# stm233/image-compression-for-machine

Hardware: AMD Instinct MI355X
Metric: images/sec (256x256) cnn-hyperprior (WACNN) training step (higher is better)
Workload: dtype f32; 1 GPU; cnn (WACNN N=192 M=320) train step, lambda=0.0067 MSE, batch 16/GPU synthetic 256x256, Adam lr 1e-4 + aux Adam, clip 1.0; global_batch=16, parallelism=dp1

## Files before the change

### image-compression-for-machine_amd/csrc/conv_wgrad.hip

```cpp
#include <algorithm>
#include <cmath>
#include <cstdlib>
#include "icm_common.h"

namespace icm {

#define WG_MAX_TAPS 32

int wgrad_wino_plan(const icm_wgrad_args& a, int nproblems, int* nsplit_out, int* nchunks_out);
int launch_wgrad_wino(const icm_wgrad_args* arr, int n, int nsplit, int nchunks, float* const* ws, float* const* dbias_ws,
                      hipStream_t stream);

#define WG_MAXG 32
struct WgPtrs {
  const float* gs;
  const float* gb;
  float* ws;
  float* dbias_ws;
};
struct WgDesc {
  WgPtrs g[WG_MAXG];
  long long gs_bs;
  PatchGeom pg;
  int Ca, OH, OW, act_s;
// ... 392 lines not shown
      const int a = a0 + ta * 32 + (r & 3) + 8 * (r >> 2) + 4 * h;
      if (a < d.Ca && b < pg.C)
        G.ws[(((long long)split * d.ntaps + tap) * d.Ca + a) * pg.C + b] = acc[i][r];
    }
    __builtin_amdgcn_sched_barrier(0);
  }
}

template <int TA, int TB, int WA, int WB, bool V4>
__global__ __launch_bounds__(512, 2) void wgrad_dma1_kernel(const WgDesc d) {
  extern __shared__ __attribute__((aligned(16))) float smem[];
  static_assert(TA == 3 * WA && TB == 3 * WB && (WA * WB == 1 || WA * WB == 2 || WA * WB == 4), "3 x 3 tiles per wave");
  constexpr int WK = 8 / (WA * WB);
  const PatchGeom& pg = d.pg;
  const int npx = 1 << d.lgNPX, grow = V4 ? 64 : npx + 1, brow = V4 ? 64 : pg.CS;
  const int gs_sz = TA * 32 * grow, gb_sz = TB * 32 * brow;
  const int bufsz = gs_sz + gb_sz;
  const int tid = threadIdx.x, lane = tid & 63;
  const int wave = __builtin_amdgcn_readfirstlane(tid >> 6);
  const WgPtrs G = d.g[blockIdx.y];
  int bid = blockIdx.x;
  if (d.xcd_order) bid = xcd_block_id();
  const int at = bid % d.natile; bid /= d.natile;
  const int bt = bid % d.nbtile;
  const int split = bid / d.nbtile;
  const int a0 = at * TA * 32, b0 = bt * TB * 32;
  const int niter = (d.ntiles - split + d.nsplit - 1) / d.nsplit;
  const int TWm = (1 << d.lgTW) - 1, THm = (1 << d.lgTH) - 1;
  const int OHW = d.OH * d.OW;
  const long long HW = (long long)pg.H * pg.W;
  const float* zero = icm_zero_page + lane;
  const float* zero4 = icm_zero_page + 4 * lane;

  auto stage = [&](int it) {
    int q = split + it * d.nsplit;
    const int tx_i = q % d.tiles_x; q /= d.tiles_x;
    const int ty_i = q % d.tiles_y;
    const int tn_i = q / d.tiles_y;
    const int ox0 = tx_i << d.lgTW, oy0 = ty_i << d.lgTH, n0 = tn_i << d.lgTI;
    float* gsT = smem + (it & 1) * bufsz;
    float* gbP = gsT + gs_sz;
    const int tx = lane & TWm, ty = (lane >> d.lgTW) & THm, ti = lane >> (d.lgTW + d.lgTH);
    const int n = n0 + ti, oy = oy0 + ty, ox = ox0 + tx;
    const bool pv = n < pg.N && oy < d.OH && ox < d.OW;
    const float* abase = G.gs + ((long long)n * d.gs_bs + oy * d.OW + ox);
    const float* bbase = G.gb + ((long long)n * pg.bs + oy * pg.W + ox);
    if constexpr (V4) {
      const int s = lane >> 4, q = lane & 15;
      for (int i = wave; i < (TA + TB) * 8; i += 8) {
        const bool isa = i < TA * 8;
        const int r = (isa ? i : i - TA * 8) * 4 + s;
        const int px = ((q - (r & 15)) & 15) * 4;
        const int tx4 = px & TWm, ty4 = (px >> d.lgTW) & THm, ti4 = px >> (d.lgTW + d.lgTH);
        const int n4 = n0 + ti4, oy4 = oy0 + ty4, ox4 = ox0 + tx4;
        const bool pv4 = n4 < pg.N && oy4 < d.OH && ox4 < d.OW;
        const float* src;
        if (isa) {
          const int a = a0 + r;
          src = (pv4 && a < d.Ca) ? G.gs + ((long long)n4 * d.gs_bs + (long long)a * OHW + oy4 * d.OW + ox4) : zero4;
        } else {
          const int c = b0 + r;
          src = (pv4 && c < pg.C) ? G.gb + ((long long)n4 * pg.bs + (long long)c * HW + oy4 * pg.W + ox4) : zero4;
        }
        __builtin_amdgcn_global_load_lds(src, (isa ? gsT : gbP) + (isa ? i : i - TA * 8) * 256, 16, 0, 0);
      }
    } else if (lane < npx) {
      for (int r = wave; r < TA * 32; r += 8) {
        const int a = a0 + r;
        __builtin_amdgcn_global_load_lds((pv && a < d.Ca) ? abase + (long long)a * OHW : zero, gsT + r * grow, 4, 0, 0);
      }
      for (int r = wave; r < TB * 32; r += 8) {
        const int c = b0 + r;
        __builtin_amdgcn_global_load_lds((pv && c < pg.C) ? bbase + (long long)c * HW : zero, gbP + r * pg.CS, 4, 0, 0);
      }
    }
  };

  const int h = lane >> 5, l31 = lane & 31;
  const int wk = wave % WK, wsp = wave / WK;
  const int wa = wsp / WB, wb = wsp % WB;
  int boffs[3];
#pragma unroll
  for (int u = 0; u < 3; ++u) boffs[u] = ((wb * 3 + u) * 32 + l31) * brow + (V4 ? 0 : h);
  const int rot = 4 * (l31 & 15) + h;
  f32x16 acc[9];
#pragma unroll
  for (int i = 0; i < 9; ++i)
#pragma unroll
    for (int r = 0; r < 16; ++r) acc[i][r] = 0.0f;
  float bsum[3] = {0.0f, 0.0f, 0.0f};
  const int nkp = npx >> 1;

  stage(0);
  asm volatile("s_waitcnt vmcnt(0)" ::: "memory");
  __syncthreads();
  for (int it = 0; it < niter; ++it) {
    if (it + 1 < niter) stage(it + 1);
    const float* gsT = smem + (it & 1) * bufsz;
    const float* gbP = gsT + gs_sz;
    const float* arow = gsT + (wa * 3 * 32 + l31) * grow + (V4 ? 0 : h);
    float avA[3], bvA[3], avB[3], bvB[3];
    auto fetch = [&](float (&av)[3], float (&bv)[3], int kn) {
      const int col = V4 ? ((2 * kn + rot) & 63) : 2 * kn;
#pragma unroll
      for (int u = 0; u < 3; ++u) av[u] = arow[u * 32 * grow + col];
#pragma unroll
      for (int u = 0; u < 3; ++u) bv[u] = gbP[boffs[u] + col];
    };
    auto mma = [&](const float (&av)[3], const float (&bv)[3]) {
#pragma unroll
      for (int ta = 0; ta < 3; ++ta)
#pragma unroll
        for (int tb = 0; tb < 3; ++tb)
          acc[ta * 3 + tb] = __builtin_amdgcn_mfma_f32_32x32x2f32(av[ta], bv[tb], acc[ta * 3 + tb], 0, 0, 0);
#pragma unroll
      for (int u = 0; u < 3; ++u) bsum[u] += av[u];
    };
    fetch(avA, bvA, wk);
    for (int kp = wk; kp < nkp; kp += 2 * WK) {
      fetch(avB, bvB, min(kp + WK, nkp - 1));
      mma(avA, bvA);
      fetch(avA, bvA, min(kp + 2 * WK, nkp - 1));
      if (kp + WK < nkp) mma(avB, bvB);
    }
    asm volatile("s_waitcnt vmcnt(0)" ::: "memory");
    __syncthreads();
  }
  constexpr int SET = 9 * 16 * 64;
  constexpr int SLOTS = (WK - 1) < 2 ? (WK - 1) : 2;
  float* red = smem + wsp * SLOTS * SET;
#pragma unroll
  for (int r0 = 1; r0 < WK; r0 += SLOTS) {
    if (wk >= r0 && wk < r0 + SLOTS) {
      float* dst = red + (wk - r0) * SET;
#pragma unroll
      for (int i = 0; i < 9; ++i)
#pragma unroll
        for (int r = 0; r < 16; ++r) dst[(i * 16 + r) * 64 + lane] = acc[i][r];
    }
    __syncthreads();
    if (wk == 0) {
      for (int k = 0; k < SLOTS && r0 + k < WK; ++k)
#pragma unroll
        for (int i = 0; i < 9; ++i)
#pragma unroll
          for (int r = 0; r < 16; ++r) acc[i][r] += red[k * SET + (i * 16 + r) * 64 + lane];
    }
    __syncthreads();
  }
  if (G.dbias_ws != nullptr && bt == 0) {
    float* bred = smem;
    if (wb == 0) {
#pragma unroll
      for (int u = 0; u < 3; ++u) {
        const float sfull = bsum[u] + __shfl_xor(bsum[u], 32, 64);
        if (h == 0) bred[(wa * WK + wk) * 96 + u * 32 + l31] = sfull;
      }
    }
    __syncthreads();
    if (wb == 0 && wk == 0 && h == 0) {
#pragma unroll
      for (int u = 0; u < 3; ++u) {
        float t = 0.0f;
        for (int k = 0; k < WK; ++k) t += bred[(wa * WK + k) * 96 + u * 32 + l31];
        const int a = a0 + (wa * 3 + u) * 32 + l31;
        if (a < d.Ca) G.dbias_ws[(long long)split * d.Ca + a] = t;
      }
    }
  }
  if (wk != 0) return;
#pragma unroll
  for (int i = 0; i < 9; ++i) {
    const int ta = wa * 3 + i / 3, tb = wb * 3 + i % 3;
    const int b = b0 + tb * 32 + l31;
#pragma unroll
    for (int r = 0; r < 16; ++r) {
      const int a = a0 + ta * 32 + (r & 3) + 8 * (r >> 2) + 4 * h;
      if (a < d.Ca && b < pg.C) G.ws[((long long)split * d.Ca + a) * pg.C + b] = acc[i][r];
    }
    __builtin_amdgcn_sched_barrier(0);
  }
}

template <int TA, int TB, int NACC>
__global__ __launch_bounds__(512, 2) void wgrad_kernel(const WgDesc d) {
  extern __shared__ __attribute__((aligned(16))) float smem[];
  const PatchGeom& pg = d.pg;
  const int npx = 1 << d.lgNPX, grow = npx + 1;
  const int gs_sz = TA * 32 * grow, gb_sz = TB * 32 * pg.CS;
  const int bufsz = gs_sz + gb_sz;
  const int tid = threadIdx.x, lane = tid & 63, wave = tid >> 6;
  const bool loader = wave >= 4;
  const WgPtrs G = d.g[blockIdx.y];

  int bid = blockIdx.x;
  if (d.xcd_order) bid = xcd_block_id();
  const int at = bid % d.natile; bid /= d.natile;
  const int bt = bid % d.nbtile; bid /= d.nbtile;
  const int tg = bid % d.ngroups;
  const int split = bid / d.ngroups;
  const int a0 = at * TA * 32, b0 = bt * TB * 32, t0 = tg * d.tpg;
  const int nt = min(d.tpg, d.ntaps - t0);
  const int TWm = (1 << d.lgTW) - 1, THm = (1 << d.lgTH) - 1;
  const int niter = (d.ntiles - split + d.nsplit - 1) / d.nsplit;

  if (loader) {
    wgrad_loader<TA, TB>(d, G, smem, tid, lane, wave, a0, b0, split, niter, bt, tg);
    return;
  }

  const int h = lane >> 5, l31 = lane & 31;
  const int ntile = nt * TA * TB;
  int boffs[NACC];
  int tsel[NACC];
#pragma unroll
  for (int i = 0; i < NACC; ++i) {
    const int q = wave + 4 * i;
    const int qq = q < ntile ? q : 0;
    const int tap = qq / (TA * TB), rem = qq % (TA * TB);
    const int ta = rem / TB, tb = rem % TB;
    tsel[i] = q < ntile ? ta : -1;
    boffs[i] = (tb * 32 + l31) * pg.CS + d.tapoff[t0 + tap] + h * d.po_h;
  }
  f32x16 acc[NACC];
#pragma unroll
  for (int i = 0; i < NACC; ++i)
#pragma unroll
    for (int r = 0; r < 16; ++r) acc[i][r] = 0.0f;

  const int pe_lane = d.pe[lane & 31];
  constexpr bool kPerAcc = (TA * TB == 16);
  static_assert(kPerAcc ? (NACC == 4 && TA == 4) : (4 % (TA * TB) == 0), "tile -> A-row mapping");
  constexpr int NA = kPerAcc ? TA : 1;
  const int ta_w = kPerAcc ? 0 : (wave % (TA * TB)) / TB;
  __syncthreads();
  const int nkp = npx >> 1;
  for (int it = 0; it < niter; ++it) {
    const float* gsT = smem + (it & 1) * bufsz;
    const float* gbP = gsT + gs_sz;
    const float* arow = gsT + (ta_w * 32 + l31) * grow + h;
    float avA[NA], bvA[NACC], avB[NA], bvB[NACC];
    auto fetch = [&](float (&av)[NA], float (&bv)[NACC], int kn) {
      const int po = __builtin_amdgcn_readlane(pe_lane, kn);
#pragma unroll
      for (int u = 0; u < NA; ++u) av[u] = arow[u * 32 * grow + 2 * kn];
#pragma unroll
      for (int i = 0; i < NACC; ++i) bv[i] = gbP[boffs[i] + po];
    };
    auto mma = [&](const float (&av)[NA], const float (&bv)[NACC]) {
#pragma unroll
      for (int i = 0; i < NACC; ++i)
        acc[i] = __builtin_amdgcn_mfma_f32_32x32x2f32(av[kPerAcc ? i : 0], bv[i], acc[i], 0, 0, 0);
    };
    fetch(avA, bvA, 0);
    for (int kp = 0; kp < nkp; kp += 2) {
      fetch(avB, bvB, kp + 1);
      mma(avA, bvA);
#pragma unroll
      for (int i = 0; i < NACC; ++i) {
        __builtin_amdgcn_sched_group_barrier(0x008, 1, 0);
        __builtin_amdgcn_sched_group_barrier(0x002, 2, 0);
        __builtin_amdgcn_sched_group_barrier(0x100, 2, 0);
      }
      fetch(avA, bvA, min(kp + 2, nkp - 1));
      mma(avB, bvB);
#pragma unroll
      for (int i = 0; i < NACC; ++i) {
        __builtin_amdgcn_sched_group_barrier(0x008, 1, 0);
        __builtin_amdgcn_sched_group_barrier(0x002, 2, 0);
        __builtin_amdgcn_sched_group_barrier(0x100, 2, 0);
      }
    }
    __syncthreads();
  }

#pragma unroll
  for (int i = 0; i < NACC; ++i) {
    if (tsel[i] < 0) continue;
    const int q = wave + 4 * i;
    const int tap = t0 + q / (TA * TB), rem = q % (TA * TB);
    const int ta = rem / TB, tb = rem % TB;
    const int b = b0 + tb * 32 + l31;
#pragma unroll
    for (int r = 0; r < 16; ++r) {
      const int a = a0 + ta * 32 + (r & 3) + 8 * (r >> 2) + 4 * h;
      if (a < d.Ca && b < pg.C)
        G.ws[(((long long)split * d.ntaps + tap) * d.Ca + a) * pg.C + b] = acc[i][r];
    }
    __builtin_amdgcn_sched_barrier(0);
  }
}

struct RedPtrs {
  const float* ws;
  float* dw;
  const float* dbias_ws;
  float* dbias;
  int accum, accum_bias;
  int dw_ld;
};
struct RedDesc {
  RedPtrs g[WG_MAXG];
  int Ca, Cb, ntaps, nsplit, nsplit_bias, nwblocks, vec4;
  int wino;
};
__global__ __launch_bounds__(256) void wgrad_reduce_kernel(const RedDesc d) {
  __shared__ __attribute__((aligned(16))) float tile[WG_MAX_TAPS][257];
  const RedPtrs G = d.g[blockIdx.y];
  const int Ca = d.Ca, ntaps = d.ntaps, nsplit = d.nsplit;
  if ((int)blockIdx.x >= d.nwblocks) {
    if (!G.dbias) return;
    float* part = &tile[0][0];
    const int pl = threadIdx.x & 15, sl = threadIdx.x >> 4;
    const int a = ((int)blockIdx.x - d.nwblocks) * 16 + pl;
    float s = 0.0f;
    if (a < Ca)
      for (int k = sl; k < d.nsplit_bias; k += 16) s += G.dbias_ws[(long long)k * Ca + a];
    part[sl * 16 + pl] = s;
    __syncthreads();
    if (sl == 0 && a < Ca) {
      float t = part[pl];
#pragma unroll
      for (int u = 1; u < 16; ++u) t += part[u * 16 + pl];
      if (G.accum_bias) t += G.dbias[a];
      G.dbias[a] = t;
    }
    return;
  }
  const long long CaCb = (long long)Ca * d.Cb;
  const long long slab = CaCb * ntaps;
  if (d.vec4) {
    f32x4* part = reinterpret_cast<f32x4*>(&tile[0][0]);
    const int pl = threadIdx.x & 15, sl = threadIdx.x >> 4;
    const long long ab = ((long long)blockIdx.x * 16 + pl) * 4;
    f32x4 s = f32x4{0.0f, 0.0f, 0.0f, 0.0f};
    if (ab < CaCb) {
      const float* p = G.ws + ab;
      int k = sl;
      for (; k + 7 * 16 < nsplit; k += 8 * 16) {
        f32x4 v[8];
#pragma unroll
        for (int u = 0; u < 8; ++u) v[u] = *reinterpret_cast<const f32x4*>(p + (long long)(k + 16 * u) * slab);
#pragma unroll
        for (int u = 0; u < 8; ++u) s += v[u];
      }
      for (; k < nsplit; k += 16) s += *reinterpret_cast<const f32x4*>(p + (long long)k * slab);
    }
    part[sl * 16 + pl] = s;
    __syncthreads();
    if (sl == 0 && ab < CaCb) {
      f32x4 t = part[pl];
#pragma unroll
      for (int u = 1; u < 16; ++u) t += part[u * 16 + pl];
      const long long ar = ab / d.Cb;
      f32x4* o = reinterpret_cast<f32x4*>(G.dw + (G.dw_ld == d.Cb ? ab : ar * G.dw_ld + (ab - ar * d.Cb)));
      if (G.accum) t += *o;
      *o = t;
    }
    return;
  }
  const int pl = threadIdx.x & 63, tl = threadIdx.x >> 6;
  const long long ab0 = (long long)blockIdx.x * 64;
  const long long ab = ab0 + pl;
  const bool valid = ab < CaCb;
  for (int t = tl; t < ntaps; t += 8) {
    const int t2 = t + 4;
    float sa = 0.0f, sb = 0.0f;
    if (valid) {
      const float* pa = G.ws + (long long)t * CaCb + ab;
      const float* pb = G.ws + (long long)(t2 < ntaps ? t2 : t) * CaCb + ab;
      for (int k = 0; k < nsplit; k += 8) {
        float va[8], vb[8];
#pragma unroll
        for (int u = 0; u < 8; ++u) {
          va[u] = (k + u < nsplit) ? pa[(long long)(k + u) * slab] : 0.0f;
          vb[u] = (k + u < nsplit) ? pb[(long long)(k + u) * slab] : 0.0f;
        }
        sa += ((va[0] + va[1]) + (va[2] + va[3])) + ((va[4] + va[5]) + (va[6] + va[7]));
        sb += ((vb[0] + vb[1]) + (vb[2] + vb[3])) + ((vb[4] + vb[5]) + (vb[6] + vb[7]));
      }
    }
    tile[t][pl] = sa;
    if (t2 < ntaps) tile[t2][pl] = sb;
  }
  __syncthreads();
  const int nv = (int)min((long long)64, CaCb - ab0);
  if (d.wino) {
    for (int e = threadIdx.x; e < nv * 9; e += 256) {
      const int abl = e / 9, t = e - abl * 9;
      const int p = t / 3, q = t - p * 3;
      float col[4];
#pragma unroll
      for (int i = 0; i < 4; ++i) {
        const float u0 = tile[i * 4 + 0][abl], u1 = tile[i * 4 + 1][abl], u2 = tile[i * 4 + 2][abl], u3 = tile[i * 4 + 3][abl];
        col[i] = q == 0 ? u0 + 0.5f * (u1 + u2) : (q == 1 ? 0.5f * (u1 - u2) : 0.5f * (u1 + u2) + u3);
      }
      float v = p == 0 ? col[0] + 0.5f * (col[1] + col[2]) : (p == 1 ? 0.5f * (col[1] - col[2]) : 0.5f * (col[1] + col[2]) + col[3]);
      const long long abg = ab0 + abl, ar = abg / d.Cb;
      float* o = G.dw + (ar * G.dw_ld + (abg - ar * d.Cb)) * 9 + t;
      if (G.accum) v += *o;
      *o = v;
    }
    return;
  }
  if (G.dw_ld == d.Cb) {
    float* o = G.dw + ab0 * ntaps;
    for (int e = threadIdx.x; e < nv * ntaps; e += 256) {
      const int abl = e / ntaps, t = e - abl * ntaps;
      float v = tile[t][abl];
      if (G.accum) v += o[e];
      o[e] = v;
    }
  } else {
    for (int e = threadIdx.x; e < nv * ntaps; e += 256) {
      const int abl = e / ntaps, t = e - abl * ntaps;
      const long long abg = ab0 + abl, ar = abg / d.Cb;
      float* o = G.dw + (ar * G.dw_ld + (abg - ar * d.Cb)) * ntaps + t;
      float v = tile[t][abl];
      if (G.accum) v += *o;
      *o = v;
    }
  }
}

enum WgFamily {
  WG_GENERAL,
  WG_T33,
  WG_T33_TAPW,
  WG_TAP9,
  WG_TAP25,
  WG_DMA1,
};
typedef void (*WgKernel)(const WgDesc);
struct WgVariant {
  WgFamily fam;
  int ta, tb, nacc;
  int tpg;
  bool halves;
  int lds_kb;
  WgKernel fn, fn_v4;
};
static const WgVariant kWgVariants[] = {
     {WG_GENERAL, 2, 1, 7, 14, true, 150, wgrad_kernel<2, 1, 7>, nullptr},
     {WG_GENERAL, 2, 2, 9, 9, false, 150, wgrad_kernel<2, 2, 9>, nullptr},
     {WG_GENERAL, 4, 4, 4, 1, false, 150, wgrad_kernel<4, 4, 4>, nullptr},
     {WG_T33, 3, 3, 9, 1, false, 160, wgrad_t33_kernel<3, 3, 1, 1>, nullptr},
     {WG_T33, 6, 6, 9, 1, false, 160, wgrad_t33_kernel<6, 6, 2, 2>, nullptr},
     {WG_T33, 3, 6, 9, 1, false, 160, wgrad_t33_kernel<3, 6, 1, 2>, nullptr},
     {WG_T33, 6, 3, 9, 1, false, 160, wgrad_t33_kernel<6, 3, 2, 1>, nullptr},
     {WG_T33_TAPW, 3, 3, 9, 4, false, 160, wgrad_t33_kernel<3, 3, 1, 1, true>, nullptr},
     {WG_TAP9, 3, 3, 9, 9, false, 160, wgrad_tap9_kernel<3, 3>, nullptr},
     {WG_TAP9, 2, 2, 9, 9, false, 160, wgrad_tap9_kernel<2, 2>, nullptr},
     {WG_TAP25, 3, 1, 10, 25, false, 160, wgrad_tap9_kernel<3, 1, 3>, nullptr},
     {WG_DMA1, 6, 6, 9, 1, false, 160, wgrad_dma1_kernel<6, 6, 2, 2, false>, wgrad_dma1_kernel<6, 6, 2, 2, true>},
     {WG_DMA1, 3, 6, 9, 1, false, 160, wgrad_dma1_kernel<3, 6, 1, 2, false>, wgrad_dma1_kernel<3, 6, 1, 2, true>},
     {WG_DMA1, 6, 3, 9, 1, false, 160, wgrad_dma1_kernel<6, 3, 2, 1, false>, wgrad_dma1_kernel<6, 3, 2, 1, true>},
     {WG_DMA1, 3, 3, 9, 1, false, 160, wgrad_dma1_kernel<3, 3, 1, 1, false>, wgrad_dma1_kernel<3, 3, 1, 1, true>},
};
constexpr int WG_NVARIANTS = sizeof(kWgVariants) / sizeof(kWgVariants[0]);
static int g_force_variant = -1, g_force_xcd = -1;

struct WgPlan {
  int variant, tpg;
  int lgTW, lgTH, lgTI, lgNPX, PH, PW, PP, CS;
  int tiles_x, tiles_y, tiles_n, ntiles, nsplit, natile, nbtile, ngroups;
  size_t lds;
};

static size_t wg_staging_bytes(int ta, int tb, int lgNPX, int CS) {
  return (size_t)2 * (ta * 32 * ((1 << lgNPX) + 1) + tb * 32 * CS) * 4;
}
static size_t wg_fold_bytes(const WgVariant& v) {
  const int waves = v.fam == WG_T33 ? 4 : (v.fam == WG_DMA1 ? 8 : 0);
  if (!waves) return 0;
  const int groups = (v.ta / 3) * (v.tb / 3), wk = waves / groups;
  return wk > 1 ? (size_t)groups * std::min(wk - 1, 2) * 9 * 16 * 64 * 4 : 0;
}
static bool wg_admit(int vi, const icm_wgrad_args& a, WgPlan& p) {
  const WgVariant& v = kWgVariants[vi];
  const int ntaps = a.KH * a.KW;
  const bool plain = a.act_s == ICM_ACT_NONE && a.act_b == ICM_ACT_NONE;
  if (v.fam == WG_DMA1 && !(ntaps == 1 && a.stride == 1 && a.pad == 0 && plain)) return false;
  if (v.fam == WG_TAP9 && !(a.KH == 3 && a.KW == 3 && a.stride == 1 && a.pad == 1 && plain)) return false;
  if (v.fam == WG_TAP25 && !(a.KH == 5 && a.KW == 5 && a.pad == 2 && plain)) return false;
  const size_t need = std::max(wg_staging_bytes(v.ta, v.tb, p.lgNPX, p.CS), wg_fold_bytes(v));
  if (need > (size_t)v.lds_kb * 1024) return false;
  const int tpg = v.halves && ntaps > v.tpg ? (ntaps + 1) / 2 : std::min(ntaps, v.tpg);
  if (tpg > v.tpg) return false;
  p.variant = vi; p.tpg = tpg; p.lds = need;
  return true;
}
static double wg_padded_area(const icm_wgrad_args& a, int ta, int tb, double factor = 1.0) {
  return (double)cdiv(a.Ca, 32 * ta) * 32 * ta * cdiv(a.Cb, 32 * tb) * 32 * tb * factor;
}
static double wg_staging_factor(int ta, int tb) { return std::max(1.0, 5.2 * (1.0 / ta + 1.0 / tb)); }

static int plan_wgrad(const icm_wgrad_args& a, WgPlan& p, int nproblems = 1) {
  if (!a.gs || !a.gb || a.N <= 0 || a.Ca <= 0 || a.Cb <= 0 || a.KH * a.KW > WG_MAX_TAPS) return ICM_ERR_ARG;
  if (a.stride != 1 && a.stride != 2) return ICM_ERR_UNSUPPORTED;
  if (a.OH != (a.H + 2 * a.pad - a.KH) / a.stride + 1 || a.OW != (a.W + 2 * a.pad - a.KW) / a.stride + 1)
    return ICM_ERR_ARG;
  const int ntaps = a.KH * a.KW;
  bool ok = false;
  for (int lg = 6; lg >= 4 && !ok; --lg) {
    p.lgNPX = lg;
    const bool halo_free = a.KH == 1 && a.KW == 1 && a.stride == 1 && a.pad == 0;
    p.lgTW = std::min(std::min(halo_free ? lg : 4, lg), ceil_log2(a.OW));
    p.lgTH = std::min(lg - p.lgTW, ceil_log2(a.OH));
    p.lgTI = lg - p.lgTW - p.lgTH;
    const int TW = 1 << p.lgTW, TH = 1 << p.lgTH, TI = 1 << p.lgTI;
    p.PW = (TW - 1) * a.stride + a.KW;
    p.PH = (TH - 1) * a.stride + a.KH;
    p.PP = p.PH * p.PW;
    p.CS = TI * p.PP;
    if ((p.CS & 1) == 0) p.CS += 1;
    auto variant = [&](int v) { return wg_admit(v, a, p); };
    if (g_force_variant >= 0) ok = variant(g_force_variant);
    else if (ntaps == 1) {
      static const int cand[] = {4, 5, 6, 3, 2};
      double bestc = 1e300;
      int bestv = -1;
      for (const int v : cand) {
        const WgVariant& c = kWgVariants[v];
        if (wg_staging_bytes(c.ta, c.tb, lg, p.CS) > 160 * 1024) continue;
        const double cost = wg_padded_area(a, c.ta, c.tb, wg_staging_factor(c.ta, c.tb));
        if (cost < bestc - 1e-9) { bestc = cost; bestv = v; }
      }
      ok = bestv >= 0 && variant(bestv);
      static const int dma1_on = env_int("ICM_WG_DMA1", 1);
      if (ok && dma1_on && a.act_s == ICM_ACT_NONE && a.act_b == ICM_ACT_NONE && a.stride == 1 && a.pad == 0) {
        static const int dc[] = {13, 12, 11, 14};
        double ba = 1e300;
        int bv = -1;
        for (const int v : dc) {
          const double area = wg_padded_area(a, kWgVariants[v].ta, kWgVariants[v].tb);
          if (area < ba - 1e-9) {
            WgPlan keep = p;
            if (variant(v)) { ba = area; bv = v; }
            p = keep;
          }
        }
        if (bv >= 0) variant(bv);
      }
      if (ok && lg == 6 && kWgVariants[p.variant].fam != WG_DMA1) {
        const WgVariant& c = kWgVariants[p.variant];
        const double area6 = wg_padded_area(a, c.ta, c.tb, wg_staging_factor(c.ta, c.tb));
        const double area66 = wg_padded_area(a, 6, 6, std::max(1.0, 5.2 / 3.0));
        if (area66 < area6 - 1e-9) ok = false;
      }
    }
    else if (ntaps <= 9 && wg_staging_bytes(2, 2, lg, p.CS) <= 150 * 1024) {
      const double pad64 = wg_padded_area(a, 2, 2);
      const double pad96 = wg_padded_area(a, 3, 3, 4.0 * cdiv(ntaps, 4) / ntaps);
      static const int tap9_on = env_int("ICM_WG_TAP9", 1);
      const double p96 = wg_padded_area(a, 3, 3);
      ok = tap9_on && ntaps == 9 && p96 <= pad64 && (long long)a.N * a.OH * a.OW >= 16384 && variant(8);
      if (!ok) ok = (ntaps > 1 && pad96 * 1.1 < pad64 && variant(7)) || variant(1);
    }
    else {
      static const int tap25_on = env_int("ICM_WG_TAP25", 1);
      ok = tap25_on && ntaps == 25 && (long long)a.N * a.OH * a.OW >= 16384 && variant(10);
      if (ok && TI * p.PP > ICM_MAXJ * 64) ok = false;
      if (!ok) ok = variant(0);
    }
    if (ok && TI * p.PP > ICM_MAXJ * 64) ok = false;
  }
  if (!ok) return ICM_ERR_UNSUPPORTED;
  const WgVariant& v = kWgVariants[p.variant];
  const int TW = 1 << p.lgTW, TH = 1 << p.lgTH, TI = 1 << p.lgTI;
  p.tiles_x = cdiv(a.OW, TW); p.tiles_y = cdiv(a.OH, TH); p.tiles_n = cdiv(a.N, TI);
  p.ntiles = p.tiles_x * p.tiles_y * p.tiles_n;
  p.natile = cdiv(a.Ca, 32 * v.ta); p.nbtile = cdiv(a.Cb, 32 * v.tb); p.ngroups = cdiv(ntaps, p.tpg);
  const int base = p.natile * p.nbtile * p.ngroups * std::max(1, nproblems);
  const int occ = std::max<int>(1, std::min<int>(2, (int)((160 * 1024) / p.lds)));
  const double slots = 256.0 * occ;
  double best = 1e300;
  p.nsplit = 1;
  for (int sp = 1; sp <= std::min(p.ntiles, 256); ++sp) {
    const double rounds = std::ceil((double)base * sp / slots);
    const double per = (double)cdiv(p.ntiles, sp) + 0.8;
    const double cost = rounds * per * (1.0 + 0.004 * sp);
    if (cost < best - 1e-9) { best = cost; p.nsplit = sp; }
  }
  return ICM_OK;
}

static long long slab_floats(int nsplit, int taps_in_slab, int Ca, int Cb) { return (long long)nsplit * taps_in_slab * Ca * Cb; }
static long long workspace_floats(int nsplit, int taps_in_slab, int Ca, int Cb) {
  return slab_floats(nsplit, taps_in_slab, Ca, Cb) + (long long)nsplit * Ca;
}
static bool members_agree(const icm_wgrad_args* arr, int n) {
  const icm_wgrad_args& a = arr[0];
  for (int i = 0; i < n; ++i) {
    const icm_wgrad_args& b = arr[i];
    if (!b.gs || !b.gb || !b.dw || !b.ws) return false;
    if (b.Ca != a.Ca || b.Cb != a.Cb || b.OH != a.OH || b.OW != a.OW || b.H != a.H || b.W != a.W || b.N != a.N ||
        b.KH != a.KH || b.KW != a.KW || b.stride != a.stride || b.pad != a.pad || b.act_s != a.act_s ||
        b.act_b != a.act_b || b.gs_bs != a.gs_bs || b.gb_bs != a.gb_bs || b.algo != a.algo)
      return false;
  }
  return true;
}
static bool workspaces_fit(const icm_wgrad_args* arr, int n, long long need) {
  for (int i = 0; i < n; ++i)
    if (arr[i].ws_floats > 0 && arr[i].ws_floats < need) return false;
  return true;
}
static int fill_reduce(RedDesc& r, const icm_wgrad_args* arr, int n, int nsplit, int taps_in_slab, int wino) {
  const icm_wgrad_args& a = arr[0];
  const long long slab_all = slab_floats(nsplit, taps_in_slab, a.Ca, a.Cb), CaCb = (long long)a.Ca * a.Cb;
  bool v4 = taps_in_slab == 1 && (CaCb % 4) == 0;
  for (int i = 0; i < WG_MAXG; ++i) {
    const icm_wgrad_args& b = arr[i < n ? i : 0];
    r.g[i].ws = b.ws; r.g[i].dw = b.dw; r.g[i].dbias_ws = b.dbias ? b.ws + slab_all : nullptr; r.g[i].dbias = b.dbias;
    r.g[i].accum = b.accum; r.g[i].accum_bias = b.accum_bias;
    r.g[i].dw_ld = b.dw_ld > 0 ? b.dw_ld : a.Cb;
    if (r.g[i].dw_ld < a.Cb) return ICM_ERR_ARG;
    v4 = v4 && ((reinterpret_cast<uintptr_t>(b.ws) & 15) == 0) && ((reinterpret_cast<uintptr_t>(b.dw) & 15) == 0);
    if (r.g[i].dw_ld != a.Cb) v4 = v4 && (a.Cb % 4) == 0 && (r.g[i].dw_ld % 4) == 0;
  }
  r.Ca = a.Ca; r.Cb = a.Cb; r.ntaps = taps_in_slab; r.nsplit = nsplit; r.nsplit_bias = nsplit; r.wino = wino;
  r.vec4 = v4 ? 1 : 0;
  r.nwblocks = (int)((CaCb + 63) / 64);
  return ICM_OK;
}
static int launch_reduce(const RedDesc& r, const icm_wgrad_args* arr, int n, hipStream_t stream) {
  bool any_bias = false;
  for (int i = 0; i < n; ++i) any_bias |= arr[i].dbias != nullptr;
  const int rblocks = r.nwblocks + (any_bias ? cdiv(r.Ca, 16) : 0);
  hipLaunchKernelGGL(wgrad_reduce_kernel, dim3(rblocks, n), dim3(256), 0, stream, r);
  ICM_CHECK_LAUNCH();
  return ICM_OK;
}

static int wgrad_wino_grouped(const icm_wgrad_args* arr, int n, hipStream_t stream) {
  const icm_wgrad_args* a = &arr[0];
  int nsplit = 0, nchunks = 0;
  if (!a->gs || !a->gb || a->N <= 0 || a->Ca <= 0 || a->Cb <= 0) return ICM_ERR_ARG;
  int rc = wgrad_wino_plan(*a, n, &nsplit, &nchunks);
  if (rc) return rc;
  if ((long long)a->N * ((a->W + 1) / 2) * ((a->H + 1) / 2) >= 65536) return ICM_ERR_UNSUPPORTED;
  if (!members_agree(arr, n) || !workspaces_fit(arr, n, workspace_floats(nsplit, 16, a->Ca, a->Cb))) return ICM_ERR_ARG;
  const long long slab_all = slab_floats(nsplit, 16, a->Ca, a->Cb);
  float* wsp[WG_MAXG];
  float* dbp[WG_MAXG];
  for (int i = 0; i < n; ++i) {
    wsp[i] = arr[i].ws;
    dbp[i] = arr[i].dbias ? arr[i].ws + slab_all : nullptr;
  }
  rc = launch_wgrad_wino(arr, n, nsplit, nchunks, wsp, dbp, stream);
  if (rc) return rc;
  RedDesc r{};
  rc = fill_reduce(r, arr, n, nsplit, 16, 1);
  return rc ? rc : launch_reduce(r, arr, n, stream);
}

static int wgrad_direct_grouped(const icm_wgrad_args* arr, int n, hipStream_t stream) {
  const icm_wgrad_args* a = &arr[0];
  WgPlan p;
  int rc = plan_wgrad(*a, p, n);
  if (rc) return rc;
  if (!members_agree(arr, n)) return ICM_ERR_ARG;
  if (((long long)a->N * a->gb_bs + 8LL * a->H * a->W) * 4 >= (1LL << 31)) return ICM_ERR_UNSUPPORTED;
  const WgVariant& v = kWgVariants[p.variant];
  const int ntaps = a->KH * a->KW;
  if (!workspaces_fit(arr, n, workspace_floats(p.nsplit, ntaps, a->Ca, a->Cb))) return ICM_ERR_ARG;
  WgDesc d{};
  RedDesc r{};
  rc = fill_reduce(r, arr, n, p.nsplit, ntaps, 0);
  if (rc) return rc;
  const long long slab_all = slab_floats(p.nsplit, ntaps, a->Ca, a->Cb);
  for (int i = 0; i < WG_MAXG; ++i) {
    const icm_wgrad_args& b = arr[i < n ? i : 0];
    d.g[i].gs = b.gs; d.g[i].gb = b.gb; d.g[i].ws = b.ws; d.g[i].dbias_ws = b.dbias ? b.ws + slab_all : nullptr;
  }
  d.gs_bs = a->gs_bs;
  PatchGeom& pg = d.pg;
  pg.PW = p.PW; pg.PH = p.PH; pg.PWrow = p.PW; pg.PWh = 0; pg.PP = p.PP; pg.CS = p.CS; pg.S = 1;
  pg.TIPH = (1 << p.lgTI) * p.PH;
  pg.dPW = make_fastdiv((uint32_t)p.PW);
  pg.dTIPH = make_fastdiv((uint32_t)pg.TIPH);
  pg.dPH = make_fastdiv((uint32_t)p.PH);
  pg.H = a->H; pg.W = a->W; pg.N = a->N; pg.C = a->Cb; pg.act = a->act_b; pg.bs = a->gb_bs;
  pg.seg_len = 0; pg.seg_gap = 0; pg.dseg = make_fastdiv(1);
  {
    const int TW = 1 << p.lgTW;
    bool v4 = ntaps == 1 && a->stride == 1 && a->pad == 0 && p.lgNPX >= 5 && (TW % 4) == 0 && (a->W % 4) == 0 &&
              (a->gb_bs % 4) == 0 && ((long long)a->H * a->W % 4) == 0 && (p.PW % 4) == 0 && (p.PP % 4) == 0;
    bool g4 = p.lgNPX >= 5 && (TW % 4) == 0 && (a->OW % 4) == 0 && (a->gs_bs % 4) == 0 &&
              ((long long)a->OH * a->OW % 4) == 0;
    for (int i = 0; i < n; ++i) {
      v4 = v4 && ((reinterpret_cast<uintptr_t>(arr[i].gb) & 15) == 0);
      g4 = g4 && ((reinterpret_cast<uintptr_t>(arr[i].gs) & 15) == 0);
    }
    pg.vec4 = v4 ? 1 : 0;
    set_v4_pack(pg);
    d.gs_vec4 = g4 ? 1 : 0;
    static const int dma_on = env_int("ICM_WG_DMA", 1);
    pg.dma = (dma_on && (a->act_b == ICM_ACT_NONE || dma_on > 1) && !v4) ? 1 : 0;
    static const int pipe_on = env_int("ICM_WG_PIPE", 1);
    pg.pipe = pipe_on;
  }
  d.Ca = a->Ca; d.OH = a->OH; d.OW = a->OW; d.act_s = a->act_s;
  d.xcd_order = ((long long)a->N * a->OH * a->OW >= 16384) ? 1 : 0;
  if (g_force_xcd >= 0) d.xcd_order = g_force_xcd;
  d.S = a->stride; d.pad = a->pad; d.ntaps = ntaps; d.tpg = p.tpg;
  d.lgTW = p.lgTW; d.lgTH = p.lgTH; d.lgTI = p.lgTI; d.lgNPX = p.lgNPX;
  d.tiles_x = p.tiles_x; d.tiles_y = p.tiles_y; d.tiles_n = p.tiles_n; d.ntiles = p.ntiles; d.nsplit = p.nsplit;
  d.natile = p.natile; d.nbtile = p.nbtile; d.ngroups = p.ngroups;
  for (int t = 0; t < WG_MAX_TAPS; ++t) d.tapoff[t] = 0;
  for (int kh = 0; kh < a->KH; ++kh)
    for (int kw = 0; kw < a->KW; ++kw) d.tapoff[kh * a->KW + kw] = kh * p.PW + kw;
  {
    const int TWm = (1 << p.lgTW) - 1, THm = (1 << p.lgTH) - 1;
    auto off = [&](int px) {
      const int tx = px & TWm, ty = (px >> p.lgTW) & THm, ti = px >> (p.lgTW + p.lgTH);
      return ti * p.PP + ty * a->stride * p.PW + tx * a->stride;
    };
    for (int kp = 0; kp < 32; ++kp) d.pe[kp] = (2 * kp < (1 << p.lgNPX)) ? off(2 * kp) : 0;
    d.po_h = off(1) - off(0);
  }
  const long long nblk = (long long)p.natile * p.nbtile * p.ngroups * p.nsplit;
  static const bool dma1_v4_off = env_int("ICM_WG_DMA1_V4", 1) == 0;
  bool v4dma = !dma1_v4_off && v.fam == WG_DMA1 && p.lgNPX == 6 && p.lgTW >= 2 && (a->OW % 4) == 0 &&
               (a->gs_bs % 4) == 0 && (a->gb_bs % 4) == 0;
  for (int i = 0; i < n && v4dma; ++i)
    v4dma = ((reinterpret_cast<uintptr_t>(arr[i].gs) | reinterpret_cast<uintptr_t>(arr[i].gb)) & 15) == 0;
  const WgKernel fn = v4dma ? v.fn_v4 : v.fn;
  if (p.lds > 64 * 1024 && !ensure_max_lds(reinterpret_cast<const void*>(fn))) return ICM_ERR_LAUNCH;
  hipLaunchKernelGGL(fn, dim3((unsigned)nblk, n), dim3(512), p.lds, stream, d);
  ICM_CHECK_LAUNCH();
  return launch_reduce(r, arr, n, stream);
}

}

extern "C" {

int64_t icm_wgrad_workspace_floats_grouped(const icm_wgrad_args* a, int n) {
  if (a && n >= 1 && a->algo == ICM_ALGO_WINOGRAD) {
    int nsplit = 0, nchunks = 0;
    if (!a->gs || !a->gb || a->N <= 0 || a->Ca <= 0 || a->Cb <= 0 || icm::wgrad_wino_plan(*a, n, &nsplit, &nchunks)) return -1;
    return icm::workspace_floats(nsplit, 16, a->Ca, a->Cb);
  }
  icm::WgPlan p;
  if (!a || n < 1 || icm::plan_wgrad(*a, p, n)) return -1;
  return icm::workspace_floats(p.nsplit, a->KH * a->KW, a->Ca, a->Cb);
}
int64_t icm_wgrad_workspace_floats(const icm_wgrad_args* a) { return icm_wgrad_workspace_floats_grouped(a, 1); }

static int wgrad_grouped(const icm_wgrad_args* arr, int n, hipStream_t stream) {
  if (!arr || n < 1 || n > WG_MAXG) return ICM_ERR_ARG;
  if (arr[0].algo == ICM_ALGO_WINOGRAD) return icm::wgrad_wino_grouped(arr, n, stream);
  if (arr[0].algo != ICM_ALGO_DIRECT) return ICM_ERR_ARG;
  return icm::wgrad_direct_grouped(arr, n, stream);
}

void icm_debug_force_wgrad_cfg(int variant, int xcd_order) {
  icm::g_force_variant = (variant >= 0 && variant < icm::WG_NVARIANTS) ? variant : -1;
  icm::g_force_xcd = (xcd_order == 0 || xcd_order == 1) ? xcd_order : -1;
}

int icm_debug_wgrad_plan(const icm_wgrad_args* a, int n, int32_t out[8]) {
  for (int i = 0; i < 8; ++i) out[i] = 0;
  if (!a || n < 1) return ICM_ERR_ARG;
  icm::WgPlan p;
  const int rc = icm::plan_wgrad(*a, p, n);
  if (rc) return rc;
  const int32_t vals[8] = {p.variant, p.lgNPX, p.lgTW, p.lgTH, p.lgTI, p.tpg, p.nsplit, (int32_t)p.lds};
  for (int i = 0; i < 8; ++i) out[i] = vals[i];
  return ICM_OK;
}

int icm_conv_wgrad(const icm_wgrad_args* a, void* stream_) {
  return wgrad_grouped(a, 1, (hipStream_t)stream_);
}
int icm_conv_wgrad_grouped(const icm_wgrad_args* arr, int n, void* stream_) {
  return wgrad_grouped(arr, n, (hipStream_t)stream_);
}

}
```

### image-compression-for-machine_amd/csrc/wgrad_wino.hip

```cpp
#include <algorithm>
#include <cmath>
#include <cstdlib>
#include <type_traits>
#include "icm_common.h"

namespace icm {

#define WW_MAXG 32
#define WW_ROW 68
#define WW_SIDE (16 * 8 * WW_ROW)
#define WW_BUF (2 * WW_SIDE)

typedef float f32x2 __attribute__((ext_vector_type(2)));
typedef float f32x2u __attribute__((ext_vector_type(2), aligned(4)));
typedef float f32x4u __attribute__((ext_vector_type(4), aligned(4)));

template <int I, int N, class F>
__device__ __forceinline__ void ww_static_for(F&& f) {
  if constexpr (I < N) {
    f(std::integral_constant<int, I>{});
    ww_static_for<I + 1, N>(f);
  }
}

struct WwPtrs {
  const float* gs;
  const float* gb;
  float* ws;
  float* dbias_ws;
};
struct WwDesc {
  WwPtrs g[WW_MAXG];
  long long gs_bs, gb_bs;
  int N, Ca, Cb, H, W, act_s, act_b;
  int TW, TH;
  FastDiv dTW, dTH;
  int ntiles, nchunks, nsplit, natile, nbtile;
};

template <bool VEC>
__global__ __launch_bounds__(512, 2) void wgrad_wino_kernel(const WwDesc d) {
  extern __shared__ __attribute__((aligned(16))) float smem[];
  const int tid = threadIdx.x, lane = tid & 63;
  const int wave = __builtin_amdgcn_readfirstlane(tid >> 6);
  const WwPtrs G = d.g[blockIdx.y];
  int bid = blockIdx.x;
  const int at = bid % d.natile; bid /= d.natile;
  const int bt = bid % d.nbtile;
  const int split = bid / d.nbtile;
  const int a0 = at * 64, b0 = bt * 64;
  const int niter = (d.nchunks - split + d.nsplit - 1) / d.nsplit;
  const int HW = d.H * d.W;

  const int ch_l = wave * 8 + (lane >> 3), tl = lane & 7;
  const bool aok = a0 + ch_l < d.Ca, bok = b0 + ch_l < d.Cb;
  const int offa = (a0 + ch_l) * HW, offb = (b0 + ch_l) * HW;
  float bsum = 0.0f;

  f32x2 ya[2];
  f32x4 xb[4];
  unsigned vmask = 0;
  unsigned oa_cur = 0, ob_cur = 0;
  auto prep = [&](int it) {
    const int tau = (split + it * d.nsplit) * 8 + tl;
    const uint32_t q = fdiv((uint32_t)tau, d.dTW);
    const int tx = tau - (int)q * d.TW;
    const uint32_t n = fdiv(q, d.dTH);
    const int ty = (int)(q - n * (uint32_t)d.TH);
    const bool tok = tau < d.ntiles;
    const int oy = ty * 2, ox = tx * 2;
    oa_cur = (unsigned)(offa + (int)n * (int)d.gs_bs + oy * d.W + ox);
    unsigned m = 0;
    if constexpr (VEC) {
#pragma unroll
      for (int r = 0; r < 2; ++r) m |= (unsigned)(tok && aok && oy + r < d.H) << r;
#pragma unroll
      for (int r = 0; r < 4; ++r) m |= (unsigned)(tok && bok && (unsigned)(oy - 1 + r) < (unsigned)d.H) << (2 + r);
      const bool left = ox == 0, right = ox == d.W - 2;
      m |= (unsigned)left << 8 | (unsigned)right << 9;
      ob_cur = (unsigned)(offb + (int)n * (int)d.gb_bs + (oy - 1) * d.W + (ox - 1) + (left ? 1 : (right ? -1 : 0)));
    } else {
#pragma unroll
      for (int r = 0; r < 2; ++r)
#pragma unroll
        for (int c = 0; c < 2; ++c) m |= (unsigned)(tok && aok && oy + r < d.H && ox + c < d.W) << (2 * r + c);
#pragma unroll
      for (int r = 0; r < 4; ++r)
#pragma unroll
        for (int c = 0; c < 4; ++c)
          m |= (unsigned)(tok && bok && (unsigned)(oy - 1 + r) < (unsigned)d.H && (unsigned)(ox - 1 + c) < (unsigned)d.W) << (4 + 4 * r + c);
      ob_cur = (unsigned)(offb + (int)n * (int)d.gb_bs + (oy - 1) * d.W + (ox - 1));
    }
    vmask = m;
  };
  auto piece = [&](auto kc) {
    constexpr int k = decltype(kc)::value;
    if constexpr (k < 2) {
      constexpr int r = k;
      if constexpr (VEC) {
        const unsigned off = (vmask >> r & 1u) ? oa_cur + r * d.W : 0u;
        const f32x2u v = *reinterpret_cast<const f32x2u*>(G.gs + off);
        ya[r] = f32x2{v[0], v[1]};
      } else {
#pragma unroll
        for (int c = 0; c < 2; ++c) ya[r][c] = G.gs[(vmask >> (2 * r + c) & 1u) ? oa_cur + r * d.W + c : 0u];
      }
    } else {
      constexpr int r = k - 2;
      if constexpr (VEC) {
        const unsigned off = (vmask >> (2 + r) & 1u) ? ob_cur + r * d.W : 0u;
        const f32x4u v = *reinterpret_cast<const f32x4u*>(G.gb + off);
        xb[r] = f32x4{v[0], v[1], v[2], v[3]};
      } else {
#pragma unroll
        for (int c = 0; c < 4; ++c) xb[r][c] = G.gb[(vmask >> (4 + 4 * r + c) & 1u) ? ob_cur + r * d.W + c : 0u];
      }
    }
  };
  float tY[4][2], uX[16];
  auto rowpass = [&]() {
    {
      float y[4];
#pragma unroll
      for (int r = 0; r < 2; ++r)
#pragma unroll
        for (int c = 0; c < 2; ++c) y[2 * r + c] = (vmask >> (VEC ? r : 2 * r + c) & 1u) ? ya[r][c] : 0.0f;
      bsum += (y[0] + y[1]) + (y[2] + y[3]);
#pragma unroll
      for (int c = 0; c < 2; ++c) {
        tY[0][c] = y[0 * 2 + c];
        tY[1][c] = y[0 * 2 + c] + y[1 * 2 + c];
        tY[2][c] = y[0 * 2 + c] - y[1 * 2 + c];
        tY[3][c] = -y[1 * 2 + c];
      }
    }
    {
      float dd[16];
      if constexpr (VEC) {
        const bool left = vmask >> 8 & 1u, right = vmask >> 9 & 1u;
#pragma unroll
        for (int r = 0; r < 4; ++r) {
          const bool rok = vmask >> (2 + r) & 1u;
          const f32x4 v = xb[r];
          const float e0 = left ? 0.0f : (right ? v[1] : v[0]);
          const float e1 = left ? v[0] : (right ? v[2] : v[1]);
          const float e2 = left ? v[1] : (right ? v[3] : v[2]);
          const float e3 = left ? v[2] : (right ? 0.0f : v[3]);
          dd[r * 4 + 0] = rok ? e0 : 0.0f;
          dd[r * 4 + 1] = rok ? e1 : 0.0f;
          dd[r * 4 + 2] = rok ? e2 : 0.0f;
          dd[r * 4 + 3] = rok ? e3 : 0.0f;
        }
      } else {
#pragma unroll
        for (int r = 0; r < 4; ++r)
#pragma unroll
          for (int c = 0; c < 4; ++c) dd[r * 4 + c] = (vmask >> (4 + 4 * r + c) & 1u) ? xb[r][c] : 0.0f;
      }
#pragma unroll
      for (int j = 0; j < 4; ++j) {
        uX[0 * 4 + j] = dd[0 * 4 + j] - dd[2 * 4 + j];
        uX[1 * 4 + j] = dd[1 * 4 + j] + dd[2 * 4 + j];
        uX[2 * 4 + j] = dd[2 * 4 + j] - dd[1 * 4 + j];
        uX[3 * 4 + j] = dd[1 * 4 + j] - dd[3 * 4 + j];
      }
    }
  };
  auto store_part = [&](auto gc, int buf) {
    constexpr int g = decltype(gc)::value;
    float* da = smem + buf * WW_BUF + tl * WW_ROW + ch_l;
    if constexpr (g < 4) {
      constexpr int i = g;
      da[(i * 4 + 0) * 8 * WW_ROW] = tY[i][0];
      da[(i * 4 + 1) * 8 * WW_ROW] = tY[i][0] + tY[i][1];
      da[(i * 4 + 2) * 8 * WW_ROW] = tY[i][0] - tY[i][1];
      da[(i * 4 + 3) * 8 * WW_ROW] = -tY[i][1];
    } else {
      constexpr int i = g - 4;
      float* db = da + WW_SIDE;
      db[(i * 4 + 0) * 8 * WW_ROW] = uX[i * 4 + 0] - uX[i * 4 + 2];
      db[(i * 4 + 1) * 8 * WW_ROW] = uX[i * 4 + 1] + uX[i * 4 + 2];
      db[(i * 4 + 2) * 8 * WW_ROW] = uX[i * 4 + 2] - uX[i * 4 + 1];
      db[(i * 4 + 3) * 8 * WW_ROW] = uX[i * 4 + 1] - uX[i * 4 + 3];
    }
  };

  const int h = lane >> 5, l31 = lane & 31;
  f32x16 acc[2][2][2];
#pragma unroll
  for (int x = 0; x < 2; ++x)
#pragma unroll
    for (int i = 0; i < 2; ++i)
#pragma unroll
      for (int j = 0; j < 2; ++j)
#pragma unroll
        for (int e = 0; e < 16; ++e) acc[x][i][j][e] = 0.0f;
  const int foff = (2 * wave) * 8 * WW_ROW + h * WW_ROW + l31;
  auto multiply = [&](int rd, int wr) {
    const float* pa = smem + rd * WW_BUF + foff;
    const float* pb = pa + WW_SIDE;
    float a0v = pa[0], a1v = pa[32], b0v = pb[0], b1v = pb[32];
    ww_static_for<0, 8>([&](auto gc) {
      constexpr int g = decltype(gc)::value, x = g >> 2;
      float na0 = 0.0f, na1 = 0.0f, nb0 = 0.0f, nb1 = 0.0f;
      if constexpr (g < 7) {
        constexpr int o = (((g + 1) >> 2) * 8 + 2 * ((g + 1) & 3)) * WW_ROW;
        na0 = pa[o]; na1 = pa[o + 32]; nb0 = pb[o]; nb1 = pb[o + 32];
      }
      if constexpr (g < 3) {
        piece(std::integral_constant<int, 2 * g>{});
        piece(std::integral_constant<int, 2 * g + 1>{});
      }
      store_part(gc, wr);
      __builtin_amdgcn_sched_barrier(0);
      acc[x][0][0] = __builtin_amdgcn_mfma_f32_32x32x2f32(a0v, b0v, acc[x][0][0], 0, 0, 0);
      acc[x][0][1] = __builtin_amdgcn_mfma_f32_32x32x2f32(a0v, b1v, acc[x][0][1], 0, 0, 0);
      acc[x][1][0] = __builtin_amdgcn_mfma_f32_32x32x2f32(a1v, b0v, acc[x][1][0], 0, 0, 0);
      acc[x][1][1] = __builtin_amdgcn_mfma_f32_32x32x2f32(a1v, b1v, acc[x][1][1], 0, 0, 0);
      __builtin_amdgcn_sched_barrier(0);
      a0v = na0; a1v = na1; b0v = nb0; b1v = nb1;
    });
  };

  prep(0);
  ww_static_for<0, 6>(piece);
  rowpass();
  ww_static_for<0, 8>([&](auto gc) { store_part(gc, 0); });
  prep(1);
  ww_static_for<0, 6>(piece);
  __syncthreads();
  for (int it = 0; it < niter; ++it) {
    rowpass();
    prep(it + 2);
    multiply(it & 1, (it + 1) & 1);
    __syncthreads();
  }

  if (G.dbias_ws != nullptr && bt == 0) {
    float s = bsum;
    s += __shfl_xor(s, 1, 64);
    s += __shfl_xor(s, 2, 64);
    s += __shfl_xor(s, 4, 64);
    if (tl == 0 && aok) G.dbias_ws[(long long)split * d.Ca + a0 + ch_l] = s;
  }
#pragma unroll
  for (int x = 0; x < 2; ++x) {
    const int xi = 2 * wave + x;
#pragma unroll
    for (int i = 0; i < 2; ++i)
#pragma unroll
      for (int j = 0; j < 2; ++j) {
        const int b = b0 + j * 32 + l31;
        float* row0 = G.ws + (((long long)split * 16 + xi) * d.Ca + a0 + i * 32 + 4 * h) * d.Cb + b;
#pragma unroll
        for (int e = 0; e < 16; ++e) {
          const int ar = (e & 3) + 8 * (e >> 2);
          if (a0 + i * 32 + 4 * h + ar < d.Ca && b < d.Cb) row0[(long long)ar * d.Cb] = acc[x][i][j][e];
        }
        __builtin_amdgcn_sched_barrier(0);
      }
  }
}

int wgrad_wino_plan(const icm_wgrad_args& a, int nproblems, int* nsplit_out, int* nchunks_out) {
  if (a.KH != 3 || a.KW != 3 || a.stride != 1 || a.pad != 1 || a.OH != a.H || a.OW != a.W) return ICM_ERR_UNSUPPORTED;
  if (a.act_s != ICM_ACT_NONE || a.act_b != ICM_ACT_NONE) return ICM_ERR_UNSUPPORTED;
  const int TW = cdiv(a.W, 2), TH = cdiv(a.H, 2);
  const long long ntiles = (long long)a.N * TW * TH;
  if (ntiles >= 65536) return ICM_ERR_UNSUPPORTED;
  if ((long long)a.N * a.gs_bs + (long long)(a.Ca + 64) * a.H * a.W >= (1LL << 30) ||
      (long long)a.N * a.gb_bs + (long long)(a.Cb + 64) * a.H * a.W >= (1LL << 30))
    return ICM_ERR_UNSUPPORTED;
  const int nchunks = (int)((ntiles + 7) / 8);
  const int base = cdiv(a.Ca, 64) * cdiv(a.Cb, 64) * std::max(1, nproblems);
  double best = 1e300;
  int nsplit = 1;
  for (int sp = 1; sp <= std::min(nchunks, 256); ++sp) {
    const double rounds = std::ceil((double)base * sp / 256.0);
    const double per = (double)cdiv(nchunks, sp) + 2.0;
    const double cost = rounds * per * (1.0 + 0.004 * sp);
    if (cost < best - 1e-9) { best = cost; nsplit = sp; }
  }
  *nsplit_out = nsplit;
  *nchunks_out = nchunks;
  return ICM_OK;
}

int launch_wgrad_wino(const icm_wgrad_args* arr, int n, int nsplit, int nchunks, float* const* ws, float* const* dbias_ws,
                      hipStream_t stream) {
  const icm_wgrad_args& a = arr[0];
  WwDesc d{};
  for (int i = 0; i < WW_MAXG; ++i) {
    const int k = i < n ? i : 0;
    d.g[i].gs = arr[k].gs; d.g[i].gb = arr[k].gb; d.g[i].ws = ws[k]; d.g[i].dbias_ws = dbias_ws[k];
  }
  d.gs_bs = a.gs_bs; d.gb_bs = a.gb_bs;
  d.N = a.N; d.Ca = a.Ca; d.Cb = a.Cb; d.H = a.H; d.W = a.W; d.act_s = a.act_s; d.act_b = a.act_b;
  d.TW = cdiv(a.W, 2); d.TH = cdiv(a.H, 2);
  d.dTW = make_fastdiv((uint32_t)d.TW); d.dTH = make_fastdiv((uint32_t)d.TH);
  d.ntiles = a.N * d.TW * d.TH; d.nchunks = nchunks; d.nsplit = nsplit;
  d.natile = cdiv(a.Ca, 64); d.nbtile = cdiv(a.Cb, 64);
  const long long nblk = (long long)d.natile * d.nbtile * nsplit;
  if (nblk <= 0 || nblk > 0x7fffffffLL) return ICM_ERR_ARG;
  const size_t lds = (size_t)2 * WW_BUF * sizeof(float);
  static const bool novec = env_int("ICM_WW_NOVEC", 0) != 0;
  auto fn = (!novec && a.W % 2 == 0 && a.W >= 4) ? wgrad_wino_kernel<true> : wgrad_wino_kernel<false>;
  if (!ensure_max_lds(reinterpret_cast<const void*>(fn))) return ICM_ERR_LAUNCH;
  hipLaunchKernelGGL(fn, dim3((unsigned)nblk, n), dim3(512), lds, stream, d);
  ICM_CHECK_LAUNCH();
  return ICM_OK;
}

}
```

Before: 388.3 images/s.

## Apply Winograd output transform inside wgrad kernel before writing split partials

```diff
diff --git a/image-compression-for-machine_amd/csrc/conv_wgrad.hip b/image-compression-for-machine_amd/csrc/conv_wgrad.hip
--- a/image-compression-for-machine_amd/csrc/conv_wgrad.hip
+++ b/image-compression-for-machine_amd/csrc/conv_wgrad.hip
@@ -718,7 +718,6 @@
 struct RedDesc {
   RedPtrs g[WG_MAXG];
   int Ca, Cb, ntaps, nsplit, nsplit_bias, nwblocks, vec4;
-  int wino;
 };
 __global__ __launch_bounds__(256) void wgrad_reduce_kernel(const RedDesc d) {
   __shared__ __attribute__((aligned(16))) float tile[WG_MAX_TAPS][257];
@@ -801,24 +800,6 @@
   }
   __syncthreads();
   const int nv = (int)min((long long)64, CaCb - ab0);
-  if (d.wino) {
-    for (int e = threadIdx.x; e < nv * 9; e += 256) {
-      const int abl = e / 9, t = e - abl * 9;
-      const int p = t / 3, q = t - p * 3;
-      float col[4];
-#pragma unroll
-      for (int i = 0; i < 4; ++i) {
-        const float u0 = tile[i * 4 + 0][abl], u1 = tile[i * 4 + 1][abl], u2 = tile[i * 4 + 2][abl], u3 = tile[i * 4 + 3][abl];
-        col[i] = q == 0 ? u0 + 0.5f * (u1 + u2) : (q == 1 ? 0.5f * (u1 - u2) : 0.5f * (u1 + u2) + u3);
-      }
-      float v = p == 0 ? col[0] + 0.5f * (col[1] + col[2]) : (p == 1 ? 0.5f * (col[1] - col[2]) : 0.5f * (col[1] + col[2]) + col[3]);
-      const long long abg = ab0 + abl, ar = abg / d.Cb;
-      float* o = G.dw + (ar * G.dw_ld + (abg - ar * d.Cb)) * 9 + t;
-      if (G.accum) v += *o;
-      *o = v;
-    }
-    return;
-  }
   if (G.dw_ld == d.Cb) {
     float* o = G.dw + ab0 * ntaps;
     for (int e = threadIdx.x; e < nv * ntaps; e += 256) {
@@ -1022,7 +1003,7 @@
     if (arr[i].ws_floats > 0 && arr[i].ws_floats < need) return false;
   return true;
 }
-static int fill_reduce(RedDesc& r, const icm_wgrad_args* arr, int n, int nsplit, int taps_in_slab, int wino) {
+static int fill_reduce(RedDesc& r, const icm_wgrad_args* arr, int n, int nsplit, int taps_in_slab) {
   const icm_wgrad_args& a = arr[0];
   const long long slab_all = slab_floats(nsplit, taps_in_slab, a.Ca, a.Cb), CaCb = (long long)a.Ca * a.Cb;
   bool v4 = taps_in_slab == 1 && (CaCb % 4) == 0;
@@ -1035,7 +1016,7 @@
     v4 = v4 && ((reinterpret_cast<uintptr_t>(b.ws) & 15) == 0) && ((reinterpret_cast<uintptr_t>(b.dw) & 15) == 0);
     if (r.g[i].dw_ld != a.Cb) v4 = v4 && (a.Cb % 4) == 0 && (r.g[i].dw_ld % 4) == 0;
   }
-  r.Ca = a.Ca; r.Cb = a.Cb; r.ntaps = taps_in_slab; r.nsplit = nsplit; r.nsplit_bias = nsplit; r.wino = wino;
+  r.Ca = a.Ca; r.Cb = a.Cb; r.ntaps = taps_in_slab; r.nsplit = nsplit; r.nsplit_bias = nsplit;
   r.vec4 = v4 ? 1 : 0;
   r.nwblocks = (int)((CaCb + 63) / 64);
   return ICM_OK;
@@ -1056,8 +1037,8 @@
   int rc = wgrad_wino_plan(*a, n, &nsplit, &nchunks);
   if (rc) return rc;
   if ((long long)a->N * ((a->W + 1) / 2) * ((a->H + 1) / 2) >= 65536) return ICM_ERR_UNSUPPORTED;
-  if (!members_agree(arr, n) || !workspaces_fit(arr, n, workspace_floats(nsplit, 16, a->Ca, a->Cb))) return ICM_ERR_ARG;
-  const long long slab_all = slab_floats(nsplit, 16, a->Ca, a->Cb);
+  if (!members_agree(arr, n) || !workspaces_fit(arr, n, workspace_floats(nsplit, 9, a->Ca, a->Cb))) return ICM_ERR_ARG;
+  const long long slab_all = slab_floats(nsplit, 9, a->Ca, a->Cb);
   float* wsp[WG_MAXG];
   float* dbp[WG_MAXG];
   for (int i = 0; i < n; ++i) {
@@ -1067,7 +1048,7 @@
   rc = launch_wgrad_wino(arr, n, nsplit, nchunks, wsp, dbp, stream);
   if (rc) return rc;
   RedDesc r{};
-  rc = fill_reduce(r, arr, n, nsplit, 16, 1);
+  rc = fill_reduce(r, arr, n, nsplit, 9);
   return rc ? rc : launch_reduce(r, arr, n, stream);
 }
 
@@ -1083,7 +1064,7 @@
   if (!workspaces_fit(arr, n, workspace_floats(p.nsplit, ntaps, a->Ca, a->Cb))) return ICM_ERR_ARG;
   WgDesc d{};
   RedDesc r{};
-  rc = fill_reduce(r, arr, n, p.nsplit, ntaps, 0);
+  rc = fill_reduce(r, arr, n, p.nsplit, ntaps);
   if (rc) return rc;
   const long long slab_all = slab_floats(p.nsplit, ntaps, a->Ca, a->Cb);
   for (int i = 0; i < WG_MAXG; ++i) {
@@ -1157,7 +1138,7 @@
   if (a && n >= 1 && a->algo == ICM_ALGO_WINOGRAD) {
     int nsplit = 0, nchunks = 0;
     if (!a->gs || !a->gb || a->N <= 0 || a->Ca <= 0 || a->Cb <= 0 || icm::wgrad_wino_plan(*a, n, &nsplit, &nchunks)) return -1;
-    return icm::workspace_floats(nsplit, 16, a->Ca, a->Cb);
+    return icm::workspace_floats(nsplit, 9, a->Ca, a->Cb);
   }
   icm::WgPlan p;
   if (!a || n < 1 || icm::plan_wgrad(*a, p, n)) return -1;
diff --git a/image-compression-for-machine_amd/csrc/wgrad_wino.hip b/image-compression-for-machine_amd/csrc/wgrad_wino.hip
--- a/image-compression-for-machine_amd/csrc/wgrad_wino.hip
+++ b/image-compression-for-machine_amd/csrc/wgrad_wino.hip
@@ -243,22 +243,44 @@
     s += __shfl_xor(s, 4, 64);
     if (tl == 0 && aok) G.dbias_ws[(long long)split * d.Ca + a0 + ch_l] = s;
   }
-#pragma unroll
-  for (int x = 0; x < 2; ++x) {
-    const int xi = 2 * wave + x;
-#pragma unroll
-    for (int i = 0; i < 2; ++i)
+  const int bcol = b0 + lane;
+#pragma unroll
+  for (int i = 0; i < 2; ++i) {
+    if (a0 + i * 32 >= d.Ca) break;
+    if (i) __syncthreads();
+#pragma unroll
+    for (int x = 0; x < 2; ++x)
 #pragma unroll
       for (int j = 0; j < 2; ++j) {
-        const int b = b0 + j * 32 + l31;
-        float* row0 = G.ws + (((long long)split * 16 + xi) * d.Ca + a0 + i * 32 + 4 * h) * d.Cb + b;
-#pragma unroll
-        for (int e = 0; e < 16; ++e) {
-          const int ar = (e & 3) + 8 * (e >> 2);
-          if (a0 + i * 32 + 4 * h + ar < d.Ca && b < d.Cb) row0[(long long)ar * d.Cb] = acc[x][i][j][e];
+        float* st = smem + ((2 * wave + x) * 32 + 4 * h) * WW_ROW + j * 32 + l31;
+#pragma unroll
+        for (int e = 0; e < 16; ++e) st[((e & 3) + 8 * (e >> 2)) * WW_ROW] = acc[x][i][j][e];
+      }
+    __syncthreads();
+#pragma unroll
+    for (int k = 0; k < 4; ++k) {
+      const int ar = wave + 8 * k, a = a0 + i * 32 + ar;
+      const float* ld = smem + ar * WW_ROW + lane;
+      float col[4][3];
+#pragma unroll
+      for (int r = 0; r < 4; ++r) {
+        const float u0 = ld[(r * 4 + 0) * 32 * WW_ROW], u1 = ld[(r * 4 + 1) * 32 * WW_ROW];
+        const float u2 = ld[(r * 4 + 2) * 32 * WW_ROW], u3 = ld[(r * 4 + 3) * 32 * WW_ROW];
+        col[r][0] = u0 + 0.5f * (u1 + u2);
+        col[r][1] = 0.5f * (u1 - u2);
+        col[r][2] = 0.5f * (u1 + u2) + u3;
+      }
+      if (a < d.Ca && bcol < d.Cb) {
+        float* o = G.ws + (((long long)split * 9) * d.Ca + a) * d.Cb + bcol;
+        const long long tap = (long long)d.Ca * d.Cb;
+#pragma unroll
+        for (int q = 0; q < 3; ++q) {
+          o[(0 * 3 + q) * tap] = col[0][q] + 0.5f * (col[1][q] + col[2][q]);
+          o[(1 * 3 + q) * tap] = 0.5f * (col[1][q] - col[2][q]);
+          o[(2 * 3 + q) * tap] = 0.5f * (col[1][q] + col[2][q]) + col[3][q];
         }
-        __builtin_amdgcn_sched_barrier(0);
-      }
+      }
+    }
   }
 }
 
```

Result: no change. 391.2 images/s (median of 6 runs) (+0.7%).
